# chan0park/node2vec-by-ecc

Measured on AMD Instinct MI355X. Metric: walk-steps/s, higher is better.
Workload: dtype f64 alias draw / int32 ids (walk); f32 (SGNS)

## Files before the change

### node2vec-by-ecc_amd/csrc/n2v_sgns.hip

```cpp
#include <cmath>
#include <cstdlib>
#include <mutex>

#include "n2v_common.h"

#pragma clang fp contract(fast)

namespace {

constexpr int kExpTableSize = 1000;
constexpr float kMaxExp = 6.0f;
__constant__ float c_exp_table[kExpTableSize];

constexpr uint64_t kLcgA = 25214903917ULL, kLcgC = 11ULL, kLcgMask = (1ULL << 48) - 1;

struct SgnsArgs {
    const int32_t* walks;
    const int32_t* lens;
    int64_t n_walks;
    int32_t walk_stride;
    float* syn0;
    float* syn1neg;
    int32_t row_stride;
    int32_t window, negative;
    const uint32_t* sample_int;
    const uint32_t* cum_table;
    const uint32_t* lut;
    int32_t lut_shift;
    float alpha0, min_alpha;
    int64_t sent_base, sent_step, sent_total, alpha_batch;
    uint64_t seed, walk_id_base;
    unsigned long long* pair_count;
    unsigned long long* work;
    int32_t lpad;
    int32_t splits;
    int32_t predraw;
    const int64_t* dyn;
    int32_t dyn_sub, dyn_subs;
    int64_t dyn_n_sub_total, dyn_n_local, dyn_shard_offset;
};

__device__ __forceinline__ void resolve_span(SgnsArgs& a) {
    if (!a.dyn) return;
    const int64_t epoch_base = a.dyn[1];
    const int64_t s = a.dyn[0] * a.dyn_subs + a.dyn_sub;
    const int64_t b = s * a.dyn_n_local / a.dyn_n_sub_total, e = (s + 1) * a.dyn_n_local / a.dyn_n_sub_total;
    a.n_walks = e - b;
    a.walks += b * a.walk_stride;
    if (a.lens) a.lens += b;
    a.sent_base = epoch_base + b * a.sent_step;
    a.walk_id_base = (uint64_t)(epoch_base + a.dyn_shard_offset + b);
}

__device__ __forceinline__ uint64_t lcg_skip(uint64_t x, uint64_t k) {
    uint64_t cur_m = kLcgA, cur_c = kLcgC, acc_m = 1, acc_c = 0;
    while (k) {
        if (k & 1) { acc_m = (acc_m * cur_m) & kLcgMask; acc_c = (acc_c * cur_m + cur_c) & kLcgMask; }
        cur_c = ((cur_m + 1) * cur_c) & kLcgMask;
        cur_m = (cur_m * cur_m) & kLcgMask;
        k >>= 1;
    }
    return (acc_m * x + acc_c) & kLcgMask;
}

__device__ __forceinline__ uint64_t mix64(uint64_t x) {
    x ^= x >> 30; x *= 0xbf58476d1ce4e5b9ULL;
    x ^= x >> 27; x *= 0x94d049bb133111ebULL;
    x ^= x >> 31;
    return x;
}
__device__ __forceinline__ uint32_t hash32(uint64_t seed, uint64_t walk, uint32_t pos, uint32_t salt) {
    return (uint32_t)(mix64(seed ^ mix64(walk * 0x9E3779B97F4A7C15ULL + (((uint64_t)salt << 32) | pos))) >> 32);
}

__device__ __forceinline__ float xor_dpp1(float v) {
    return __builtin_bit_cast(float, __builtin_amdgcn_mov_dpp(__builtin_bit_cast(int, v), 0xB1, 0xf, 0xf, true));
}
__device__ __forceinline__ float xor_dpp2(float v) {
    return __builtin_bit_cast(float, __builtin_amdgcn_mov_dpp(__builtin_bit_cast(int, v), 0x4E, 0xf, 0xf, true));
}
template <int M>
__device__ __forceinline__ float xor_swz(float v) {
    return __builtin_bit_cast(float, __builtin_amdgcn_ds_swizzle(__builtin_bit_cast(int, v), (M << 10) | 0x1f));
}

__device__ __forceinline__ float reduce8(const float (&p)[8], int lane) {
    const bool b0 = lane & 1, b1 = lane & 2, b2 = lane & 4;
    float q[4], r[2];
#pragma unroll
    for (int k = 0; k < 4; ++k) {
        const float send = b0 ? p[k] : p[k + 4];
        const float keep = b0 ? p[k + 4] : p[k];
        q[k] = keep + xor_dpp1(send);
    }
#pragma unroll
    for (int k = 0; k < 2; ++k) {
        const float send = b1 ? q[k] : q[k + 2];
        const float keep = b1 ? q[k + 2] : q[k];
        r[k] = keep + xor_dpp2(send);
    }
    float s = (b2 ? r[1] : r[0]) + xor_swz<4>(b2 ? r[0] : r[1]);
    s += xor_swz<8>(s);
    s += xor_swz<16>(s);
    s += __shfl_xor(s, 32);
    return s;
}

__device__ __forceinline__ constexpr int bitrev3(int k) { return ((k & 1) << 2) | (k & 2) | ((k >> 2) & 1); }

__device__ __forceinline__ int32_t draw_target(const uint32_t* __restrict__ cum, const uint32_t* __restrict__ lut,
                                               int shift, uint32_t r) {
    const uint32_t b = r >> shift;
    uint32_t lo = lut[b], hi = lut[b + 1];
    while (lo < hi) {
        const uint32_t mid = (lo + hi) >> 1;
        if (cum[mid] < r) lo = mid + 1;
        else hi = mid;
    }
    return (int32_t)lo;
}

template <int VPL>
struct Row {
    float v[VPL];
};

enum : int { kPlain = 0, kAgent = 1, kAtomic = 2 };

template <int MODE>
__device__ __forceinline__ float2 ld2(const float* p) {
    if constexpr (MODE == kPlain) {
        return *reinterpret_cast<const float2*>(p);
    } else {
        const uint64_t b = __hip_atomic_load(reinterpret_cast<const uint64_t*>(p), __ATOMIC_RELAXED,
                                             __HIP_MEMORY_SCOPE_AGENT);
        return make_float2(__builtin_bit_cast(float, (uint32_t)b), __builtin_bit_cast(float, (uint32_t)(b >> 32)));
    }
}
template <int MODE>
__device__ __forceinline__ void st2(float* p, float x, float y) {
    if constexpr (MODE == kPlain) {
        *reinterpret_cast<float2*>(p) = make_float2(x, y);
    } else {
        const uint64_t b = (uint64_t)__builtin_bit_cast(uint32_t, x) | ((uint64_t)__builtin_bit_cast(uint32_t, y) << 32);
        __hip_atomic_store(reinterpret_cast<uint64_t*>(p), b, __ATOMIC_RELAXED, __HIP_MEMORY_SCOPE_AGENT);
    }
}

template <int VPL>
__device__ __forceinline__ int lane_off(int lane) { return VPL <= 2 ? lane * VPL : lane * 4; }

template <int VPL, int MODE>
__device__ __forceinline__ Row<VPL> load_row(const float* base, int64_t row, int stride, int lane) {
    Row<VPL> r;
    if constexpr (MODE == kAtomic) {
        const float* q = base + row * stride + lane;
#pragma unroll
        for (int i = 0; i < VPL; ++i) r.v[i] = __hip_atomic_load(q + i * 64, __ATOMIC_RELAXED, __HIP_MEMORY_SCOPE_AGENT);
        return r;
    }
    const float* p = base + row * stride + lane_off<VPL>(lane);
    if constexpr (VPL == 1) {
        if constexpr (MODE == kPlain) r.v[0] = *p;
        else r.v[0] = __hip_atomic_load(p, __ATOMIC_RELAXED, __HIP_MEMORY_SCOPE_AGENT);
    } else if constexpr (VPL == 2) {
        const float2 t = ld2<MODE>(p);
        r.v[0] = t.x; r.v[1] = t.y;
    } else {
#pragma unroll
        for (int i = 0; i < VPL; i += 4) {
            if constexpr (MODE == kPlain) {
                const float4 t = *reinterpret_cast<const float4*>(p + i * 64);
                r.v[i] = t.x; r.v[i + 1] = t.y; r.v[i + 2] = t.z; r.v[i + 3] = t.w;
            } else {
                const float2 t0 = ld2<MODE>(p + i * 64), t1 = ld2<MODE>(p + i * 64 + 2);
                r.v[i] = t0.x; r.v[i + 1] = t0.y; r.v[i + 2] = t1.x; r.v[i + 3] = t1.y;
            }
        }
    }
    return r;
}

template <int VPL, int MODE>
__device__ __forceinline__ void store_row(float* base, int64_t row, int stride, int lane, const Row<VPL>& r) {
    float* p = base + row * stride + lane_off<VPL>(lane);
    if constexpr (VPL == 1) {
        if constexpr (MODE == kPlain) *p = r.v[0];
        else __hip_atomic_store(p, r.v[0], __ATOMIC_RELAXED, __HIP_MEMORY_SCOPE_AGENT);
    } else if constexpr (VPL == 2) {
        st2<MODE>(p, r.v[0], r.v[1]);
    } else {
#pragma unroll
        for (int i = 0; i < VPL; i += 4) {
            if constexpr (MODE == kPlain) {
                *reinterpret_cast<float4*>(p + i * 64) = make_float4(r.v[i], r.v[i + 1], r.v[i + 2], r.v[i + 3]);
            } else {
                st2<MODE>(p + i * 64, r.v[i], r.v[i + 1]);
                st2<MODE>(p + i * 64 + 2, r.v[i + 2], r.v[i + 3]);
            }
        }
    }
}

template <int VPL>
__device__ __forceinline__ void add_row(float* base, int64_t row, int stride, int lane, const Row<VPL>& d) {
    float* q = base + row * stride + lane;
#pragma unroll
    for (int i = 0; i < VPL; ++i)
        __hip_atomic_fetch_add(q + i * 64, d.v[i], __ATOMIC_RELAXED, __HIP_MEMORY_SCOPE_AGENT);
}

template <int VPL>
__device__ __forceinline__ void add_row_packed(float* base, int64_t row, int stride, int lane, const Row<VPL>& d) {
    float* p = base + row * stride + lane_off<VPL>(lane);
    if constexpr (VPL <= 2) {
#pragma unroll
        for (int v = 0; v < VPL; ++v) __hip_atomic_fetch_add(p + v, d.v[v], __ATOMIC_RELAXED, __HIP_MEMORY_SCOPE_AGENT);
    } else {
#pragma unroll
        for (int i = 0; i < VPL; i += 4)
#pragma unroll
            for (int v = 0; v < 4; ++v)
                __hip_atomic_fetch_add(p + i * 64 + v, d.v[i + v], __ATOMIC_RELAXED, __HIP_MEMORY_SCOPE_AGENT);
    }
}

template <int VPL>
__device__ __forceinline__ float negative_gradient(const Row<VPL>& h, const Row<VPL>& n, float alpha) {
    float acc = 0.f;
#pragma unroll
    for (int v = 0; v < VPL; ++v) acc = fmaf(h.v[v], n.v[v], acc);
    acc += xor_dpp1(acc);
    acc += xor_dpp2(acc);
    acc += xor_swz<4>(acc);
    acc += xor_swz<8>(acc);
    acc += xor_swz<16>(acc);
    acc += __shfl_xor(acc, 32);
    const float f = __builtin_bit_cast(float, __builtin_amdgcn_readfirstlane(__builtin_bit_cast(int, acc)));
    if (!(f > -kMaxExp && f < kMaxExp)) return 0.f;
    return (0.f - c_exp_table[(int)((f + kMaxExp) * (float)(kExpTableSize / (int)kMaxExp / 2))]) * alpha;
}

__device__ __forceinline__ int64_t next_item(unsigned long long* counter, int lane) {
    unsigned long long v = 0;
    if (lane == 0) v = atomicAdd(counter, 1ull);
    const int lo = __builtin_amdgcn_readfirstlane((int)(uint32_t)v), hi = __builtin_amdgcn_readfirstlane((int)(uint32_t)(v >> 32));
    return (int64_t)(((uint64_t)(uint32_t)hi << 32) | (uint32_t)lo);
}
template <int VPL, int G, int MODE>
__attribute__((amdgpu_waves_per_eu(8, 8)))
__global__ void __launch_bounds__(256) sgns_kernel(SgnsArgs a_in) {
    SgnsArgs a = a_in;
    resolve_span(a);
    extern __shared__ int32_t smem[];
    const int lane = threadIdx.x & 63;
    const int wv = __builtin_amdgcn_readfirstlane(threadIdx.x >> 6);
    int32_t* sent = smem + wv * a.lpad;
    const int64_t n_waves = (int64_t)gridDim.x * 4;
    const int my_k = bitrev3(lane & 7);
    unsigned long long pairs_done = 0;

    const int S = a.splits;
    const int64_t n_items = a.n_walks * S;
    for (int64_t item = a.work ? next_item(a.work, lane) : (int64_t)blockIdx.x * 4 + wv; item < n_items;
         item = a.work ? next_item(a.work, lane) : item + n_waves) {
        const int64_t wi = S == 1 ? item : item / S;
        const int sp = S == 1 ? 0 : (int)(item - wi * S);
        const int len = a.lens ? a.lens[wi] : a.walk_stride;
        const uint64_t wid = a.walk_id_base + (uint64_t)wi;
        int n_eff = 0;
        for (int base = 0; base < len; base += 64) {
            const int pos = base + lane;
            bool keep = false;
            int32_t tok = -1;
            if (pos < len) {
                tok = a.walks[wi * a.walk_stride + pos];
                keep = tok >= 0;
                if (keep && a.sample_int) keep = !(a.sample_int[tok] < hash32(a.seed, wid, (uint32_t)pos, 0x5AB));
            }
            const unsigned long long m = __ballot(keep);
            if (keep) sent[n_eff + __popcll(m & ((1ULL << lane) - 1ULL))] = tok;
            n_eff += __popcll(m);
        }
        __builtin_amdgcn_fence(__ATOMIC_RELEASE, "wavefront");
        __builtin_amdgcn_wave_barrier();
        __builtin_amdgcn_fence(__ATOMIC_ACQUIRE, "wavefront");

        const int64_t pushed = a.sent_base + (wi / a.alpha_batch) * a.alpha_batch * a.sent_step;
        float alpha = a.alpha0 - (a.alpha0 - a.min_alpha) * (float)((double)pushed / (double)a.sent_total);
        alpha = fmaxf(alpha, a.min_alpha);

        uint64_t lcg = mix64(a.seed ^ mix64(wid + 0x632BE59BD9B4E019ULL)) & kLcgMask;
        int i_begin = 0, i_end = n_eff;
        if (S > 1) {
            i_begin = (int)((int64_t)sp * n_eff / S);
            i_end = (int)((int64_t)(sp + 1) * n_eff / S);
            int pairs_before = 0;
            for (int base = 0; base < i_begin; base += 64) {
                const int i = base + lane;
                int np = 0;
                if (i < i_begin) {
                    const int rb = (int)(hash32(a.seed, wid, (uint32_t)i, 0xB17) % (uint32_t)a.window);
                    const int lo = max(0, i - a.window + rb), hi = min(n_eff, i + a.window + 1 - rb);
                    np = hi - lo > 1 ? hi - lo - 1 : 0;
                }
#pragma unroll
                for (int o = 32; o > 0; o >>= 1) np += __shfl_xor(np, o, 64);
                pairs_before += np;
            }
            lcg = lcg_skip(lcg, (uint64_t)pairs_before * (uint64_t)a.negative);
        }

        for (int i = i_begin; i < i_end; ++i) {
            const int32_t ci = __builtin_amdgcn_readfirstlane(sent[i]);
            const int rb = (int)(hash32(a.seed, wid, (uint32_t)i, 0xB17) % (uint32_t)a.window);
            const int lo = max(0, i - a.window + rb), hi = min(n_eff, i + a.window + 1 - rb);
            if (hi - lo <= 1) continue;
            Row<VPL> c = load_row<VPL, MODE>(a.syn1neg, ci, a.row_stride, lane);
            Row<VPL> cd;
#pragma unroll
            for (int v = 0; v < VPL; ++v) cd.v[v] = 0.f;
            const int nd = (hi - lo - 1) * a.negative;
            const bool pre = a.predraw && nd <= 128;
            int32_t drawn0 = -1, drawn1 = -1;
            if (pre) {
#pragma unroll
                for (int half = 0; half < 2; ++half) {
                    const int d = half * 64 + lane;
                    int32_t t = -1;
                    if (d < nd) {
                        const uint64_t s = lcg_skip(lcg, (uint64_t)d);
                        t = draw_target(a.cum_table, a.lut, a.lut_shift, (uint32_t)((s >> 16) % 2147483647ULL));
                        if (t == ci) t = -1;
                    }
                    if (half == 0) drawn0 = t;
                    else drawn1 = t;
                }
            }
            int pidx = 0;
            for (int j = lo; j < hi; ++j) {
                if (j == i) continue;
                const int32_t xj = __builtin_amdgcn_readfirstlane(sent[j]);
                Row<VPL> h = load_row<VPL, MODE>(a.syn0, xj, a.row_stride, lane);
                Row<VPL> work;
#pragma unroll
                for (int v = 0; v < VPL; ++v) work.v[v] = 0.f;
                for (int t0 = 0; t0 < a.negative + 1; t0 += 8) {
                    int32_t my_t = -1;
                    if (pre) {
                        const int d = min(max(pidx * a.negative + lane - 1, 0), 127);
                        const int v0 = __builtin_amdgcn_ds_bpermute((d & 63) << 2, drawn0);
                        const int v1 = __builtin_amdgcn_ds_bpermute((d & 63) << 2, drawn1);
                        if (lane >= 1 && lane <= a.negative) my_t = d < 64 ? v0 : v1;
                    } else {
                        const int tk = t0 + lane;
                        if (lane < 8 && tk >= 1 && tk <= a.negative) {
                            uint64_t s = lcg;
                            for (int d = max(t0, 1); d < tk; ++d) s = (s * kLcgA + kLcgC) & kLcgMask;
                            const uint32_t r = (uint32_t)((s >> 16) % 2147483647ULL);
                            my_t = draw_target(a.cum_table, a.lut, a.lut_shift, r);
                            if (my_t == ci) my_t = -1;
                        }
                    }
                    int32_t tgt[G];
                    Row<VPL> n[G];
                    float p[8];
#pragma unroll
                    for (int k = 0; k < G; ++k) {
                        tgt[k] = __builtin_amdgcn_readlane(my_t, k);
                        if (k == 0 && t0 == 0) tgt[k] = ci;
                    }
                    uint32_t late = 0;
#pragma unroll
                    for (int k = 1; k < G; ++k)
#pragma unroll
                        for (int k1 = 0; k1 < k; ++k1)
                            if (tgt[k] >= 0 && tgt[k] == tgt[k1]) late |= 1u << k;
#pragma unroll
                    for (int k = 0; k < G; ++k) {
                        if (k == 0 && t0 == 0) {
                            n[k] = c;
                        } else if (tgt[k] >= 0 && !(late >> k & 1)) {
                            n[k] = load_row<VPL, MODE>(a.syn1neg, tgt[k], a.row_stride, lane);
                        } else {
#pragma unroll
                            for (int v = 0; v < VPL; ++v) n[k].v[v] = 0.f;
                        }
                    }
#pragma unroll
                    for (int k = 0; k < 8; ++k) {
                        float acc = 0.f;
                        if (k < G) {
#pragma unroll
                            for (int v = 0; v < VPL; ++v) acc = fmaf(h.v[v], n[k].v[v], acc);
                        }
                        p[k] = acc;
                    }
                    const float f = reduce8(p, lane);
                    float g = 0.f;
                    if (f > -kMaxExp && f < kMaxExp) {
                        const float sig = c_exp_table[(int)((f + kMaxExp) * (float)(kExpTableSize / (int)kMaxExp / 2))];
                        const float label = (my_k == 0 && t0 == 0) ? 1.f : 0.f;
                        g = (label - sig) * alpha;
                    }
#pragma unroll
                    for (int k = 0; k < G; ++k) {
                        if (tgt[k] < 0 || (late >> k & 1)) continue;
                        const float gk = __builtin_bit_cast(
                            float, __builtin_amdgcn_readlane(__builtin_bit_cast(int, g), bitrev3(k)));
                        if (gk == 0.f) continue;
                        Row<VPL> dn;
#pragma unroll
                        for (int v = 0; v < VPL; ++v) {
                            work.v[v] = fmaf(gk, n[k].v[v], work.v[v]);
                            dn.v[v] = gk * h.v[v];
                            n[k].v[v] += dn.v[v];
                        }
                        if (k == 0 && t0 == 0) {
                            c = n[k];
#pragma unroll
                            for (int v = 0; v < VPL; ++v) cd.v[v] += dn.v[v];
                        } else if constexpr (MODE == kAtomic) {
                            add_row<VPL>(a.syn1neg, tgt[k], a.row_stride, lane, dn);
                        } else {
                            store_row<VPL, MODE>(a.syn1neg, tgt[k], a.row_stride, lane, n[k]);
                        }
                    }
                    if (late) {
#pragma unroll
                        for (int k = 1; k < G; ++k) {
                            if (!(late >> k & 1)) continue;
                            Row<VPL> r = load_row<VPL, MODE>(a.syn1neg, tgt[k], a.row_stride, lane);
                            const float gk = negative_gradient<VPL>(h, r, alpha);
                            if (gk == 0.f) continue;
                            Row<VPL> dn;
#pragma unroll
                            for (int v = 0; v < VPL; ++v) {
                                work.v[v] = fmaf(gk, r.v[v], work.v[v]);
                                dn.v[v] = gk * h.v[v];
                                r.v[v] += dn.v[v];
                            }
                            if constexpr (MODE == kAtomic) add_row<VPL>(a.syn1neg, tgt[k], a.row_stride, lane, dn);
                            else store_row<VPL, MODE>(a.syn1neg, tgt[k], a.row_stride, lane, r);
                        }
                    }
                    const int used = min(a.negative, t0 + 7) - max(t0, 1) + 1;
                    for (int d = 0; d < used; ++d) lcg = (lcg * kLcgA + kLcgC) & kLcgMask;
                }
                if constexpr (MODE == kAtomic) {
                    add_row<VPL>(a.syn0, xj, a.row_stride, lane, work);
                } else {
#pragma unroll
                    for (int v = 0; v < VPL; ++v) h.v[v] += work.v[v];
                    store_row<VPL, MODE>(a.syn0, xj, a.row_stride, lane, h);
                }
                ++pidx;
                ++pairs_done;
            }
            if constexpr (MODE == kAtomic) add_row<VPL>(a.syn1neg, ci, a.row_stride, lane, cd);
            else if constexpr (MODE == kAgent) add_row_packed<VPL>(a.syn1neg, ci, a.row_stride, lane, cd);
            else store_row<VPL, MODE>(a.syn1neg, ci, a.row_stride, lane, c);
        }
        __builtin_amdgcn_wave_barrier();
    }
    if (a.pair_count && lane == 0 && pairs_done) atomicAdd(a.pair_count, pairs_done);
}

template <int VPL, int MODE>
__global__ void __launch_bounds__(256) sgns_shared_kernel(SgnsArgs a_in) {
    SgnsArgs a = a_in;
    resolve_span(a);
    extern __shared__ int32_t smem[];
    const int lane = threadIdx.x & 63;
    const int wv = __builtin_amdgcn_readfirstlane(threadIdx.x >> 6);
    int32_t* sent = smem + wv * a.lpad;
    const int64_t n_waves = (int64_t)gridDim.x * 4;
    const int my_k = bitrev3(lane & 7);
    unsigned long long pairs_done = 0;

    for (int64_t wi = (int64_t)blockIdx.x * 4 + wv; wi < a.n_walks; wi += n_waves) {
        const int len = a.lens ? a.lens[wi] : a.walk_stride;
        const uint64_t wid = a.walk_id_base + (uint64_t)wi;
        int n_eff = 0;
        for (int base = 0; base < len; base += 64) {
            const int pos = base + lane;
            bool keep = false;
            int32_t tok = -1;
            if (pos < len) {
                tok = a.walks[wi * a.walk_stride + pos];
                keep = tok >= 0;
                if (keep && a.sample_int) keep = !(a.sample_int[tok] < hash32(a.seed, wid, (uint32_t)pos, 0x5AB));
            }
            const unsigned long long m = __ballot(keep);
            if (keep) sent[n_eff + __popcll(m & ((1ULL << lane) - 1ULL))] = tok;
            n_eff += __popcll(m);
        }
        __builtin_amdgcn_fence(__ATOMIC_RELEASE, "wavefront");
        __builtin_amdgcn_wave_barrier();
        __builtin_amdgcn_fence(__ATOMIC_ACQUIRE, "wavefront");
        const int64_t pushed = a.sent_base + (wi / a.alpha_batch) * a.alpha_batch * a.sent_step;
        float alpha = a.alpha0 - (a.alpha0 - a.min_alpha) * (float)((double)pushed / (double)a.sent_total);
        alpha = fmaxf(alpha, a.min_alpha);
        uint64_t lcg = mix64(a.seed ^ mix64(wid + 0x632BE59BD9B4E019ULL)) & kLcgMask;

        for (int i = 0; i < n_eff; ++i) {
            const int32_t ci = __builtin_amdgcn_readfirstlane(sent[i]);
            const int rb = (int)(hash32(a.seed, wid, (uint32_t)i, 0xB17) % (uint32_t)a.window);
            const int lo = max(0, i - a.window + rb), hi = min(n_eff, i + a.window + 1 - rb);
            if (hi - lo <= 1) continue;
            int32_t my_t = -1;
            if (lane >= 1 && lane <= a.negative) {
                uint64_t s = lcg;
                for (int d = 1; d < lane; ++d) s = (s * kLcgA + kLcgC) & kLcgMask;
                my_t = draw_target(a.cum_table, a.lut, a.lut_shift, (uint32_t)((s >> 16) % 2147483647ULL));
                if (my_t == ci) my_t = -1;
            }
            for (int d = 0; d < a.negative; ++d) lcg = (lcg * kLcgA + kLcgC) & kLcgMask;
            int32_t tgt[8];
            Row<VPL> n[8], dn[8];
#pragma unroll
            for (int k = 0; k < 8; ++k) {
                tgt[k] = (k == 0) ? ci : __builtin_amdgcn_readlane(my_t, k);
#pragma unroll
                for (int k2 = 1; k2 < k; ++k2)
                    if (tgt[k] >= 0 && tgt[k] == tgt[k2]) tgt[k] = -1;
                if (tgt[k] >= 0) n[k] = load_row<VPL, MODE>(a.syn1neg, tgt[k], a.row_stride, lane);
#pragma unroll
                for (int v = 0; v < VPL; ++v) {
                    if (tgt[k] < 0) n[k].v[v] = 0.f;
                    dn[k].v[v] = 0.f;
                }
            }
            for (int j = lo; j < hi; ++j) {
                if (j == i) continue;
                const int32_t xj = __builtin_amdgcn_readfirstlane(sent[j]);
                Row<VPL> h = load_row<VPL, MODE>(a.syn0, xj, a.row_stride, lane);
                float p[8];
#pragma unroll
                for (int k = 0; k < 8; ++k) {
                    float acc = 0.f;
#pragma unroll
                    for (int v = 0; v < VPL; ++v) acc = fmaf(h.v[v], n[k].v[v], acc);
                    p[k] = acc;
                }
                const float f = reduce8(p, lane);
                float g = 0.f;
                if (f > -kMaxExp && f < kMaxExp) {
                    const float sig = c_exp_table[(int)((f + kMaxExp) * (float)(kExpTableSize / (int)kMaxExp / 2))];
                    g = ((my_k == 0 ? 1.f : 0.f) - sig) * alpha;
                }
                Row<VPL> work;
#pragma unroll
                for (int v = 0; v < VPL; ++v) work.v[v] = 0.f;
#pragma unroll
                for (int k = 0; k < 8; ++k) {
                    if (tgt[k] < 0) continue;
                    const float gk = __builtin_bit_cast(
                        float, __builtin_amdgcn_readlane(__builtin_bit_cast(int, g), bitrev3(k)));
                    if (gk == 0.f) continue;
#pragma unroll
                    for (int v = 0; v < VPL; ++v) {
                        work.v[v] = fmaf(gk, n[k].v[v], work.v[v]);
                        const float d = gk * h.v[v];
                        n[k].v[v] += d;
                        dn[k].v[v] += d;
                    }
                }
                if constexpr (MODE == kAtomic) {
                    add_row<VPL>(a.syn0, xj, a.row_stride, lane, work);
                } else {
#pragma unroll
                    for (int v = 0; v < VPL; ++v) h.v[v] += work.v[v];
                    store_row<VPL, MODE>(a.syn0, xj, a.row_stride, lane, h);
                }
                ++pairs_done;
            }
#pragma unroll
            for (int k = 0; k < 8; ++k) {
                if (tgt[k] < 0) continue;
                if constexpr (MODE == kAtomic) add_row<VPL>(a.syn1neg, tgt[k], a.row_stride, lane, dn[k]);
                else store_row<VPL, MODE>(a.syn1neg, tgt[k], a.row_stride, lane, n[k]);
            }
        }
        __builtin_amdgcn_wave_barrier();
    }
    if (a.pair_count && lane == 0 && pairs_done) atomicAdd(a.pair_count, pairs_done);
}

__global__ void __launch_bounds__(256)
sgns_init_kernel(float* syn0, float* syn1neg, int64_t n_words, int32_t dim, int32_t stride, uint64_t seed) {
    const int64_t idx = (int64_t)blockIdx.x * 256 + threadIdx.x;
    const int blocks_per_row = stride / 4;
    const int64_t row = idx / blocks_per_row;
    const int cb = (int)(idx - row * blocks_per_row);
    if (row >= n_words) return;
    uint32_t rr[4];
    n2v::philox4x32_10(seed, (uint32_t)row, (uint32_t)(row >> 32), (uint32_t)cb, 0x5EEDu, rr);
    float4 o, z = make_float4(0.f, 0.f, 0.f, 0.f);
    float* po = &o.x;
#pragma unroll
    for (int t = 0; t < 4; ++t) {
        const int colx = cb * 4 + t;
        const float u = (float)(rr[t] >> 8) * (1.0f / 16777216.0f);
        po[t] = colx < dim ? (u - 0.5f) / (float)dim : 0.f;
    }
    *reinterpret_cast<float4*>(syn0 + row * stride + cb * 4) = o;
    *reinterpret_cast<float4*>(syn1neg + row * stride + cb * 4) = z;
}

__global__ void __launch_bounds__(256)
neg_lut_kernel(const uint32_t* __restrict__ cum, int64_t n_words, int shift, int64_t n_buckets, uint32_t* __restrict__ lut) {
    const int64_t b = (int64_t)blockIdx.x * 256 + threadIdx.x;
    if (b > n_buckets) return;
    const uint64_t key = (uint64_t)b << shift;
    int64_t lo = 0, hi = n_words;
    while (lo < hi) {
        const int64_t mid = (lo + hi) >> 1;
        if ((uint64_t)cum[mid] < key) lo = mid + 1;
        else hi = mid;
    }
    lut[b] = (uint32_t)lo;
}

float host_exp_table[kExpTableSize];
bool host_exp_ready = false;

void fill_exp_table() {
    if (host_exp_ready) return;
    for (int i = 0; i < kExpTableSize; ++i) {
        const float x = ((float)i / (float)kExpTableSize * 2.0f - 1.0f) * kMaxExp;
        const float e = (float)std::exp((double)x);
        host_exp_table[i] = (float)(e / (e + 1.0f));
    }
    host_exp_ready = true;
}

std::mutex exp_upload_mutex;
bool exp_uploaded[64] = {};

int upload_exp_table() {
    int dev = 0;
    hipError_t e = hipGetDevice(&dev);
    if (e != hipSuccess || dev < 0 || dev >= 64) return n2v::fail(N2V_ERR_HIP, "n2v_sgns_train: hipGetDevice: %s", hipGetErrorString(e));
    std::lock_guard<std::mutex> lock(exp_upload_mutex);
    if (exp_uploaded[dev]) return N2V_OK;
    fill_exp_table();
    e = hipMemcpyToSymbol(HIP_SYMBOL(c_exp_table), host_exp_table, sizeof(host_exp_table), 0, hipMemcpyHostToDevice);
    if (e != hipSuccess) return n2v::fail(N2V_ERR_HIP, "n2v_sgns_train: exp table upload: %s", hipGetErrorString(e));
    exp_uploaded[dev] = true;
    return N2V_OK;
}

}

extern "C" int n2v_build_neg_lut(const uint32_t* cum_table, int64_t n_words, int32_t lut_bits, uint32_t* lut,
                                 void* stream) {
    if (!cum_table || !lut || n_words <= 0 || n_words >= ((int64_t)1 << 32) || lut_bits < 1 || lut_bits > 24)
        return n2v::fail(N2V_ERR_INVALID, "n2v_build_neg_lut: bad argument (n_words %lld, lut_bits %d)",
                         (long long)n_words, (int)lut_bits);
    const int64_t nb = (int64_t)1 << lut_bits;
    hipLaunchKernelGGL(neg_lut_kernel, dim3(n2v::grid_for(nb + 1, 256)), dim3(256), 0, (hipStream_t)stream, cum_table,
                       n_words, 31 - lut_bits, nb, lut);
    return n2v::check_launch("n2v_build_neg_lut");
}

extern "C" int n2v_sgns_init(float* syn0, float* syn1neg, int64_t n_words, int32_t dim, int32_t row_stride,
                             uint64_t seed, void* stream) {
    if (!syn0 || !syn1neg || n_words < 0 || dim < 1 || row_stride < dim || (row_stride % 4) != 0)
        return n2v::fail(N2V_ERR_INVALID, "n2v_sgns_init: bad argument");
    if (n_words == 0) return N2V_OK;
    const int64_t threads = n_words * (row_stride / 4);
    hipLaunchKernelGGL(sgns_init_kernel, dim3(n2v::grid_for(threads, 256)), dim3(256), 0, (hipStream_t)stream, syn0,
                       syn1neg, n_words, dim, row_stride, seed);
    return n2v::check_launch("n2v_sgns_init");
}

namespace {
int predraw_mode(int walk_splits, int negative) {
    (void)walk_splits;
    if (negative < 1 || negative > 7) return 0;
    const char* e = getenv("N2V_SGNS_PREDRAW");
    return (e && e[0] == '0') ? 0 : 1;
}
}

namespace {
struct SpanSpec {
    const int64_t* dyn;
    int32_t sub, subs;
    int64_t n_sub_total, n_local, shard_offset;
};

static int64_t n2v_cu_count() {
    static int cus = 0;
    if (cus == 0) {
        int dev = 0, n = 0;
        if (hipGetDevice(&dev) == hipSuccess &&
            hipDeviceGetAttribute(&n, hipDeviceAttributeMultiprocessorCount, dev) == hipSuccess && n > 0) cus = n;
        else cus = 256;
    }
    return cus;
}

static int64_t default_grid(int64_t n_words, int32_t update_mode) {
    const int64_t cus = n2v_cu_count();
    int64_t cap = 3072;
    if (cap > n_words / 256) cap = n_words / 256 > 16 ? n_words / 256 : 16;
    if (update_mode != kAtomic && cap < 4 * cus) cap = 4 * cus;
    if (cap > cus) cap -= cap % cus;
    return cap;
}

int sgns_launch(const char* who, const int32_t* walks, const int32_t* lens, int64_t n_walks, int32_t walk_stride,
                float* syn0, float* syn1neg, int64_t n_words, int32_t dim, int32_t row_stride,
                int32_t window, int32_t negative, const uint32_t* sample_int,
                const uint32_t* cum_table, const uint32_t* lut, int32_t lut_bits, float alpha,
                float min_alpha, int64_t sentences_base, int64_t sentences_step,
                int64_t sentences_total, int64_t alpha_batch,
                uint64_t seed, uint64_t walk_id_base, unsigned long long* pair_count,
                int32_t update_mode, int32_t max_blocks, int32_t walk_splits, const SpanSpec& span,
                unsigned long long* work_counter, void* stream) {
    if (walk_splits < 1 || walk_splits > walk_stride)
        return n2v::fail(N2V_ERR_INVALID, "n2v_sgns_train: walk_splits %d outside [1, %d]", (int)walk_splits, (int)walk_stride);
    if (n_walks < 0 || walk_stride < 1 || n_words < 1 || dim < 1 || window < 1 || negative < 0 || negative > 64)
        return n2v::fail(N2V_ERR_INVALID, "n2v_sgns_train: bad size (walks %lld x %d, words %lld, dim %d, window %d, negative %d)",
                         (long long)n_walks, (int)walk_stride, (long long)n_words, (int)dim, (int)window, (int)negative);
    if (n_walks == 0) return N2V_OK;
    if (!walks || !syn0 || !syn1neg || (negative > 0 && (!cum_table || !lut)))
        return n2v::fail(N2V_ERR_INVALID, "n2v_sgns_train: null pointer");
    if (row_stride < dim || (row_stride % 64) != 0 || row_stride > 512)
        return n2v::fail(N2V_ERR_INVALID, "n2v_sgns_train: row_stride %d must be a multiple of 64 in [dim, 512]",
                         (int)row_stride);
    if (lut_bits < 1 || lut_bits > 24) return n2v::fail(N2V_ERR_INVALID, "n2v_sgns_train: lut_bits %d", (int)lut_bits);
    const bool share = (update_mode & N2V_SGNS_SHARE_NEGATIVES) != 0;
    const bool unchecked = (update_mode & N2V_SGNS_UNCHECKED) != 0;
    update_mode &= ~(N2V_SGNS_SHARE_NEGATIVES | N2V_SGNS_UNCHECKED);
    if (update_mode < kPlain || update_mode > kAtomic)
        return n2v::fail(N2V_ERR_INVALID, "n2v_sgns_train: update_mode %d", (int)update_mode);
    if (share && negative > 7) return n2v::fail(N2V_ERR_INVALID, "n2v_sgns_train: shared negatives need negative <= 7");
    if (share && walk_splits != 1) return n2v::fail(N2V_ERR_INVALID, "n2v_sgns_train: shared negatives need walk_splits == 1");
    if (walk_splits > 1 && update_mode != kAtomic && !unchecked)
        return n2v::fail(N2V_ERR_INVALID, "n2v_sgns_train: walk_splits > 1 needs N2V_SGNS_ATOMIC (or N2V_SGNS_UNCHECKED)");
    if (sentences_total < 1 || alpha_batch < 1 || sentences_step < 1) return n2v::fail(N2V_ERR_INVALID, "n2v_sgns_train: bad schedule");
    hipStream_t st = (hipStream_t)stream;
    if (int rc = upload_exp_table()) return rc;

    SgnsArgs a;
    a.walks = walks; a.lens = lens; a.n_walks = n_walks; a.walk_stride = walk_stride;
    a.syn0 = syn0; a.syn1neg = syn1neg; a.row_stride = row_stride;
    a.window = window; a.negative = negative; a.sample_int = sample_int;
    a.cum_table = cum_table; a.lut = lut; a.lut_shift = 31 - lut_bits;
    a.alpha0 = alpha; a.min_alpha = min_alpha;
    a.work = share ? nullptr : work_counter;
    a.sent_base = sentences_base; a.sent_step = sentences_step; a.sent_total = sentences_total;
    a.alpha_batch = alpha_batch;
    a.seed = seed; a.walk_id_base = walk_id_base; a.pair_count = pair_count;
    a.lpad = (walk_stride + 63) & ~63;
    a.splits = walk_splits;
    a.predraw = predraw_mode(walk_splits, negative);
    a.dyn = span.dyn; a.dyn_sub = span.sub; a.dyn_subs = span.subs;
    a.dyn_n_sub_total = span.n_sub_total; a.dyn_n_local = span.n_local; a.dyn_shard_offset = span.shard_offset;
    const size_t shmem = (size_t)4 * a.lpad * sizeof(int32_t);
    if (shmem > 64 * 1024) return n2v::fail(N2V_ERR_INVALID, "n2v_sgns_train: walk_stride %d too long", (int)walk_stride);
    int64_t blocks = (n_walks * walk_splits + 3) / 4;
    const int64_t cap = max_blocks > 0 ? max_blocks : default_grid(n_words, update_mode);
    if (blocks > cap) blocks = cap;
    const dim3 grid((unsigned)blocks), block(256);
    if (n_walks * walk_splits <= blocks * 4) a.work = nullptr;
    if (a.work && hipMemsetAsync(a.work, 0, sizeof(unsigned long long), st) != hipSuccess)
        return n2v::fail(N2V_ERR_HIP, "%s: resetting the work counter failed", who);
#define N2V_SGNS_LAUNCH_M(V, M)                                                            \
    if (share) hipLaunchKernelGGL((sgns_shared_kernel<V, M>), grid, block, shmem, st, a);     \
    else if (negative <= 5) hipLaunchKernelGGL((sgns_kernel<V, 6, M>), grid, block, shmem, st, a); \
    else hipLaunchKernelGGL((sgns_kernel<V, 8, M>), grid, block, shmem, st, a)
#define N2V_SGNS_LAUNCH(V)                                   \
    if (update_mode == kPlain) { N2V_SGNS_LAUNCH_M(V, kPlain); }        \
    else if (update_mode == kAgent) { N2V_SGNS_LAUNCH_M(V, kAgent); }   \
    else { N2V_SGNS_LAUNCH_M(V, kAtomic); }
    switch (row_stride / 64) {
        case 1: N2V_SGNS_LAUNCH(1); break;
        case 2: N2V_SGNS_LAUNCH(2); break;
        case 4: N2V_SGNS_LAUNCH(4); break;
        case 8: N2V_SGNS_LAUNCH(8); break;
        default:
            return n2v::fail(N2V_ERR_INVALID, "n2v_sgns_train: row_stride %d must be 64, 128, 256 or 512", (int)row_stride);
    }
    return n2v::check_launch(who);
}
}

extern "C" int n2v_sgns_train(const int32_t* walks, const int32_t* lens, int64_t n_walks, int32_t walk_stride,
                              float* syn0, float* syn1neg, int64_t n_words, int32_t dim, int32_t row_stride,
                              int32_t window, int32_t negative, const uint32_t* sample_int,
                              const uint32_t* cum_table, const uint32_t* lut, int32_t lut_bits, float alpha,
                              float min_alpha, int64_t sentences_base, int64_t sentences_step,
                              int64_t sentences_total, int64_t alpha_batch,
                              uint64_t seed, uint64_t walk_id_base, unsigned long long* pair_count,
                              int32_t update_mode, int32_t max_blocks, int32_t walk_splits,
                              unsigned long long* work_counter, void* stream) {
    return sgns_launch("n2v_sgns_train", walks, lens, n_walks, walk_stride, syn0, syn1neg, n_words, dim, row_stride, window,
                       negative, sample_int, cum_table, lut, lut_bits, alpha, min_alpha, sentences_base, sentences_step,
                       sentences_total, alpha_batch, seed, walk_id_base, pair_count, update_mode, max_blocks, walk_splits,
                       SpanSpec{nullptr, 0, 1, 1, 0, 0}, work_counter, stream);
}

extern "C" int n2v_sgns_train_span(const int32_t* walks, const int32_t* lens, int64_t n_local, int32_t walk_stride,
                                   float* syn0, float* syn1neg, int64_t n_words, int32_t dim, int32_t row_stride,
                                   int32_t window, int32_t negative, const uint32_t* sample_int,
                                   const uint32_t* cum_table, const uint32_t* lut, int32_t lut_bits, float alpha,
                                   float min_alpha, int64_t sentences_step, int64_t sentences_total, int64_t alpha_batch,
                                   uint64_t seed, unsigned long long* pair_count, int32_t update_mode, int32_t max_blocks,
                                   int32_t walk_splits, const int64_t* interval_state, int32_t sub_index,
                                   int32_t subs_per_interval, int64_t n_sub_total, int64_t shard_offset,
                                   unsigned long long* work_counter, void* stream) {
    if (!interval_state || subs_per_interval < 1 || sub_index < 0 || sub_index >= subs_per_interval || n_sub_total < subs_per_interval ||
        (n_sub_total % subs_per_interval) != 0 || n_local < 0 || shard_offset < 0)
        return n2v::fail(N2V_ERR_INVALID, "n2v_sgns_train_span: bad span (sub %d of %d, %lld sub-intervals, %lld walks)",
                         (int)sub_index, (int)subs_per_interval, (long long)n_sub_total, (long long)n_local);
    const int64_t max_walks = (n_local + n_sub_total - 1) / n_sub_total;
    if (max_walks == 0) return N2V_OK;
    return sgns_launch("n2v_sgns_train_span", walks, lens, max_walks, walk_stride, syn0, syn1neg, n_words, dim, row_stride, window,
                       negative, sample_int, cum_table, lut, lut_bits, alpha, min_alpha, 0, sentences_step, sentences_total,
                       alpha_batch, seed, 0, pair_count, update_mode, max_blocks, walk_splits,
                       SpanSpec{interval_state, sub_index, subs_per_interval, n_sub_total, n_local, shard_offset}, work_counter, stream);
}

extern "C" int32_t n2v_sgns_default_blocks(int64_t n_words, int32_t update_mode) {
    return (int32_t)default_grid(n_words < 0 ? 0 : n_words, update_mode & 3);
}
```

Baseline: 41.37 billion.

## Add per-wave LDS row cache for syn0 context rows in SGNS kernel

Adds a small per-wave LDS cache of syn0 rows (and pending deltas in atomic/agent modes) so that context words repeated within a sliding window reuse the cached row instead of reloading and rewriting global memory. Entries are flushed once they fall outside the window, when evicted, or at the end of the walk. The aim is to cut global memory traffic and atomics. In exchange it adds ballot/min bookkeeping per pair, uses more LDS, which can lower occupancy, and delays visibility of updates to other waves. The metric is walk-steps/s, so the effect depends on whether the timed path includes SGNS at all.

```diff
diff --git a/node2vec-by-ecc_amd/csrc/n2v_sgns.hip b/node2vec-by-ecc_amd/csrc/n2v_sgns.hip
--- a/node2vec-by-ecc_amd/csrc/n2v_sgns.hip
+++ b/node2vec-by-ecc_amd/csrc/n2v_sgns.hip
@@ -35,6 +35,7 @@
     int32_t lpad;
     int32_t splits;
     int32_t predraw;
+    int32_t cache_slots;
     const int64_t* dyn;
     int32_t dyn_sub, dyn_subs;
     int64_t dyn_n_sub_total, dyn_n_local, dyn_shard_offset;
@@ -241,13 +242,61 @@
     return (0.f - c_exp_table[(int)((f + kMaxExp) * (float)(kExpTableSize / (int)kMaxExp / 2))]) * alpha;
 }
 
+template <int VPL, int MODE>
+struct CacheSlot {
+    static constexpr int kView = 0, kDelta = 64 * VPL;
+    static constexpr int kFloats = 64 * VPL * (MODE == kPlain ? 1 : 2);
+};
+template <int VPL>
+__device__ __forceinline__ Row<VPL> lds_row(const float* p) {
+    Row<VPL> r;
+    if constexpr (VPL == 2) {
+        const float2 t = *reinterpret_cast<const float2*>(p);
+        r.v[0] = t.x; r.v[1] = t.y;
+    } else {
+#pragma unroll
+        for (int v = 0; v < VPL; ++v) r.v[v] = p[v];
+    }
+    return r;
+}
+template <int VPL>
+__device__ __forceinline__ void lds_put(float* p, const Row<VPL>& r) {
+    if constexpr (VPL == 2) {
+        *reinterpret_cast<float2*>(p) = make_float2(r.v[0], r.v[1]);
+    } else {
+#pragma unroll
+        for (int v = 0; v < VPL; ++v) p[v] = r.v[v];
+    }
+}
+template <int VPL, int MODE>
+__device__ __forceinline__ void cache_flush(const SgnsArgs& a, const float* cache, int s, int32_t tok, int lane) {
+    using CS = CacheSlot<VPL, MODE>;
+    const float* p = cache + s * CS::kFloats;
+    if constexpr (MODE == kAtomic) add_row<VPL>(a.syn0, tok, a.row_stride, lane, lds_row<VPL>(p + CS::kDelta));
+    else if constexpr (MODE == kAgent) add_row_packed<VPL>(a.syn0, tok, a.row_stride, lane, lds_row<VPL>(p + CS::kDelta));
+    else store_row<VPL, MODE>(a.syn0, tok, a.row_stride, lane, lds_row<VPL>(p + CS::kView));
+}
+__device__ __forceinline__ int xor_dpp1i(int v) { return __builtin_amdgcn_mov_dpp(v, 0xB1, 0xf, 0xf, true); }
+__device__ __forceinline__ int xor_dpp2i(int v) { return __builtin_amdgcn_mov_dpp(v, 0x4E, 0xf, 0xf, true); }
+template <int M>
+__device__ __forceinline__ int xor_swzi(int v) { return __builtin_amdgcn_ds_swizzle(v, (M << 10) | 0x1f); }
+__device__ __forceinline__ int wave_min(int v) {
+    v = min(v, xor_dpp1i(v));
+    v = min(v, xor_dpp2i(v));
+    v = min(v, xor_swzi<4>(v));
+    v = min(v, xor_swzi<8>(v));
+    v = min(v, xor_swzi<16>(v));
+    v = min(v, __shfl_xor(v, 32));
+    return __builtin_amdgcn_readfirstlane(v);
+}
+
 __device__ __forceinline__ int64_t next_item(unsigned long long* counter, int lane) {
     unsigned long long v = 0;
     if (lane == 0) v = atomicAdd(counter, 1ull);
     const int lo = __builtin_amdgcn_readfirstlane((int)(uint32_t)v), hi = __builtin_amdgcn_readfirstlane((int)(uint32_t)(v >> 32));
     return (int64_t)(((uint64_t)(uint32_t)hi << 32) | (uint32_t)lo);
 }
-template <int VPL, int G, int MODE>
+template <int VPL, int G, int MODE, bool CACHE>
 __attribute__((amdgpu_waves_per_eu(8, 8)))
 __global__ void __launch_bounds__(256) sgns_kernel(SgnsArgs a_in) {
     SgnsArgs a = a_in;
@@ -259,6 +308,9 @@
     const int64_t n_waves = (int64_t)gridDim.x * 4;
     const int my_k = bitrev3(lane & 7);
     unsigned long long pairs_done = 0;
+    using CS = CacheSlot<VPL, MODE>;
+    float* cache = reinterpret_cast<float*>(smem + 4 * a.lpad) + (size_t)wv * a.cache_slots * CS::kFloats + lane * VPL;
+    int32_t slot_tok = -2, slot_reach = 0x7fffffff;
 
     const int S = a.splits;
     const int64_t n_items = a.n_walks * S;
@@ -285,6 +337,7 @@
         __builtin_amdgcn_fence(__ATOMIC_RELEASE, "wavefront");
         __builtin_amdgcn_wave_barrier();
         __builtin_amdgcn_fence(__ATOMIC_ACQUIRE, "wavefront");
+        if constexpr (CACHE) slot_tok = lane < a.cache_slots ? -1 : -2;
 
         const int64_t pushed = a.sent_base + (wi / a.alpha_batch) * a.alpha_batch * a.sent_step;
         float alpha = a.alpha0 - (a.alpha0 - a.min_alpha) * (float)((double)pushed / (double)a.sent_total);
@@ -315,6 +368,15 @@
             const int32_t ci = __builtin_amdgcn_readfirstlane(sent[i]);
             const int rb = (int)(hash32(a.seed, wid, (uint32_t)i, 0xB17) % (uint32_t)a.window);
             const int lo = max(0, i - a.window + rb), hi = min(n_eff, i + a.window + 1 - rb);
+            if constexpr (CACHE) {
+                unsigned long long stale = __ballot(slot_tok >= 0 && slot_reach < i - a.window);
+                while (stale) {
+                    const int s = __ffsll(stale) - 1;
+                    stale &= stale - 1;
+                    cache_flush<VPL, MODE>(a, cache, s, __builtin_amdgcn_readlane(slot_tok, s), lane);
+                    if (lane == s) slot_tok = -1;
+                }
+            }
             if (hi - lo <= 1) continue;
             Row<VPL> c = load_row<VPL, MODE>(a.syn1neg, ci, a.row_stride, lane);
             Row<VPL> cd;
@@ -341,7 +403,26 @@
             for (int j = lo; j < hi; ++j) {
                 if (j == i) continue;
                 const int32_t xj = __builtin_amdgcn_readfirstlane(sent[j]);
-                Row<VPL> h = load_row<VPL, MODE>(a.syn0, xj, a.row_stride, lane);
+                int cs = -1;
+                bool hit = false;
+                if constexpr (CACHE) {
+                    const unsigned long long m = __ballot(slot_tok == xj);
+                    if (m) {
+                        cs = __ffsll(m) - 1;
+                        hit = true;
+                    } else if (const unsigned long long fr = __ballot(slot_tok == -1)) {
+                        cs = __ffsll(fr) - 1;
+                    } else {
+                        const int oldest = wave_min(slot_reach);
+                        if (oldest < j) {
+                            cs = __ffsll(__ballot(slot_reach == oldest)) - 1;
+                            cache_flush<VPL, MODE>(a, cache, cs, __builtin_amdgcn_readlane(slot_tok, cs), lane);
+                        }
+                    }
+                }
+                Row<VPL> h;
+                if (CACHE && hit) h = lds_row<VPL>(cache + cs * CS::kFloats + CS::kView);
+                else h = load_row<VPL, MODE>(a.syn0, xj, a.row_stride, lane);
                 Row<VPL> work;
 #pragma unroll
                 for (int v = 0; v < VPL; ++v) work.v[v] = 0.f;
@@ -447,7 +528,25 @@
                     const int used = min(a.negative, t0 + 7) - max(t0, 1) + 1;
                     for (int d = 0; d < used; ++d) lcg = (lcg * kLcgA + kLcgC) & kLcgMask;
                 }
-                if constexpr (MODE == kAtomic) {
+                if (CACHE && cs >= 0) {
+                    float* sv = cache + cs * CS::kFloats;
+                    if constexpr (MODE != kPlain) {
+                        Row<VPL> d = work;
+                        if (hit) {
+                            const Row<VPL> d0 = lds_row<VPL>(sv + CS::kDelta);
+#pragma unroll
+                            for (int v = 0; v < VPL; ++v) d.v[v] = d0.v[v] + work.v[v];
+                        }
+                        lds_put<VPL>(sv + CS::kDelta, d);
+                    }
+#pragma unroll
+                    for (int v = 0; v < VPL; ++v) h.v[v] += work.v[v];
+                    lds_put<VPL>(sv + CS::kView, h);
+                    if (lane == cs) {
+                        slot_reach = hit ? max(slot_reach, j) : j;
+                        slot_tok = xj;
+                    }
+                } else if constexpr (MODE == kAtomic) {
                     add_row<VPL>(a.syn0, xj, a.row_stride, lane, work);
                 } else {
 #pragma unroll
@@ -460,6 +559,14 @@
             if constexpr (MODE == kAtomic) add_row<VPL>(a.syn1neg, ci, a.row_stride, lane, cd);
             else if constexpr (MODE == kAgent) add_row_packed<VPL>(a.syn1neg, ci, a.row_stride, lane, cd);
             else store_row<VPL, MODE>(a.syn1neg, ci, a.row_stride, lane, c);
+        }
+        if constexpr (CACHE) {
+            unsigned long long used = __ballot(slot_tok >= 0);
+            while (used) {
+                const int s = __ffsll(used) - 1;
+                used &= used - 1;
+                cache_flush<VPL, MODE>(a, cache, s, __builtin_amdgcn_readlane(slot_tok, s), lane);
+            }
         }
         __builtin_amdgcn_wave_barrier();
     }
@@ -681,6 +788,23 @@
     if (negative < 1 || negative > 7) return 0;
     const char* e = getenv("N2V_SGNS_PREDRAW");
     return (e && e[0] == '0') ? 0 : 1;
+}
+
+constexpr size_t kRowCacheLdsBudget = 40 * 1024, kLdsLaunchLimit = 64 * 1024;
+constexpr int kRowCacheMaxSlots = 16, kRowCacheMinSlots = 4;
+int rowcache_slots(size_t sent_bytes, int32_t row_stride, int32_t update_mode, bool share) {
+    if (share || row_stride > 128) return 0;
+    const size_t slot_bytes = (size_t)4 * row_stride * sizeof(float) * (update_mode == kPlain ? 1 : 2);
+    const char* e = getenv("N2V_SGNS_ROWCACHE");
+    if (e && e[0]) {
+        const int n = atoi(e);
+        if (n <= 0) return 0;
+        const int asked = n > 32 ? 32 : n;
+        return sent_bytes + asked * slot_bytes <= kLdsLaunchLimit ? asked : 0;
+    }
+    if (sent_bytes + kRowCacheMinSlots * slot_bytes > kRowCacheLdsBudget) return 0;
+    const size_t fit = (kRowCacheLdsBudget - sent_bytes) / slot_bytes;
+    return fit > (size_t)kRowCacheMaxSlots ? kRowCacheMaxSlots : (int)fit;
 }
 }
 
@@ -760,8 +884,11 @@
     a.predraw = predraw_mode(walk_splits, negative);
     a.dyn = span.dyn; a.dyn_sub = span.sub; a.dyn_subs = span.subs;
     a.dyn_n_sub_total = span.n_sub_total; a.dyn_n_local = span.n_local; a.dyn_shard_offset = span.shard_offset;
-    const size_t shmem = (size_t)4 * a.lpad * sizeof(int32_t);
-    if (shmem > 64 * 1024) return n2v::fail(N2V_ERR_INVALID, "n2v_sgns_train: walk_stride %d too long", (int)walk_stride);
+    const size_t sent_bytes = (size_t)4 * a.lpad * sizeof(int32_t);
+    if (sent_bytes > kLdsLaunchLimit) return n2v::fail(N2V_ERR_INVALID, "n2v_sgns_train: walk_stride %d too long", (int)walk_stride);
+    a.cache_slots = rowcache_slots(sent_bytes, row_stride, update_mode, share);
+    const bool cached = a.cache_slots > 0;
+    const size_t shmem = sent_bytes + (size_t)a.cache_slots * 4 * row_stride * sizeof(float) * (update_mode == kPlain ? 1 : 2);
     int64_t blocks = (n_walks * walk_splits + 3) / 4;
     const int64_t cap = max_blocks > 0 ? max_blocks : default_grid(n_words, update_mode);
     if (blocks > cap) blocks = cap;
@@ -769,10 +896,13 @@
     if (n_walks * walk_splits <= blocks * 4) a.work = nullptr;
     if (a.work && hipMemsetAsync(a.work, 0, sizeof(unsigned long long), st) != hipSuccess)
         return n2v::fail(N2V_ERR_HIP, "%s: resetting the work counter failed", who);
+#define N2V_SGNS_LAUNCH_C(V, GG, M)                                                                             \
+    if (cached && V <= 2) hipLaunchKernelGGL((sgns_kernel<(V <= 2 ? V : 1), GG, M, true>), grid, block, shmem, st, a); \
+    else hipLaunchKernelGGL((sgns_kernel<V, GG, M, false>), grid, block, shmem, st, a)
 #define N2V_SGNS_LAUNCH_M(V, M)                                                            \
     if (share) hipLaunchKernelGGL((sgns_shared_kernel<V, M>), grid, block, shmem, st, a);     \
-    else if (negative <= 5) hipLaunchKernelGGL((sgns_kernel<V, 6, M>), grid, block, shmem, st, a); \
-    else hipLaunchKernelGGL((sgns_kernel<V, 8, M>), grid, block, shmem, st, a)
+    else if (negative <= 5) { N2V_SGNS_LAUNCH_C(V, 6, M); }                                  \
+    else { N2V_SGNS_LAUNCH_C(V, 8, M); }
 #define N2V_SGNS_LAUNCH(V)                                   \
     if (update_mode == kPlain) { N2V_SGNS_LAUNCH_M(V, kPlain); }        \
     else if (update_mode == kAgent) { N2V_SGNS_LAUNCH_M(V, kAgent); }   \
```

Result: no change. 41.46 billion (median of 3 runs) (+0.2%).
